# rareid2/Stanford_Raytracer

Hardware: AMD Instinct MI355X
Metric: ray-steps/sec (whole node) + achieved HBM GB/s vs roofline (higher is better)
Workload: dtype f64

## Files before the change

### stanford_raytracer_amd/csrc/srt_fastmath.hpp

```cpp
#pragma once
#include <hip/hip_runtime.h>

namespace srt {

constexpr double FM_PI = 3.14159265358979323846;

__device__ __forceinline__ double fdiv(double a, double b) {
  double r = __builtin_amdgcn_rcp(b);
  r = fma(fma(-b, r, 1.0), r, r);
  r = fma(fma(-b, r, 1.0), r, r);
  double q = a * r;
  return fma(fma(-b, q, a), r, q);
}

namespace fm {
__device__ __forceinline__ double sqrt_pos(double x) {
  const double y = __builtin_amdgcn_rsq(x);
  double g = x * y, h = 0.5 * y;
  const double r = fma(-h, g, 0.5);
  g = fma(g, r, g);
  h = fma(h, r, h);
  double d = fma(-g, g, x);
  g = fma(d, h, g);
  d = fma(-g, g, x);
  g = fma(d, h, g);
  return x == 0.0 ? 0.0 : g;
}
__device__ __forceinline__ void sqrt_and_inv_pos(double x, double &g_out, double &inv_out) {
  const double y = __builtin_amdgcn_rsq(x);
  double g = x * y, h = 0.5 * y;
  const double r = fma(-h, g, 0.5);
  g = fma(g, r, g);
  h = fma(h, r, h);
  double d = fma(-g, g, x);
  g = fma(d, h, g);
  d = fma(-g, g, x);
  g = fma(d, h, g);
  double inv = h + h;
  inv = fma(fma(-g, inv, 1.0), inv, inv);
  g_out = g;
  inv_out = inv;
}
__device__ __forceinline__ void sincos_0pi(double a, double &s, double &c) {
  const double PIO2_HI = 1.57079632673412561417e+00, PIO2_LO = 6.07710050650619224932e-11;
  const double kf = a > 0.75 * FM_PI ? 2.0 : (a > 0.25 * FM_PI ? 1.0 : 0.0);
  const double t = fma(-kf, PIO2_LO, fma(-kf, PIO2_HI, a));
  const double z = t * t;
  const double rs = 8.33333333332248946124e-03 + z * (-1.98412698298579493134e-04 + z * (2.75573137070700676789e-06 + z * (-2.50507602534068634195e-08 + z * 1.58969099521155010221e-10)));
  const double st = t + (z * t) * (-1.66666666666666324348e-01 + z * rs);
  const double rc = z * (4.16666666666666019037e-02 + z * (-1.38888888888741095749e-03 + z * (2.48015872894767294178e-05 + z * (-2.75573143513906633035e-07 + z * (2.08757232129817482790e-09 + z * -1.13596475577881948265e-11)))));
  const double hz = 0.5 * z, w = 1.0 - hz;
  const double ct = w + (((1.0 - w) - hz) + z * rc);
  s = kf == 1.0 ? ct : (kf == 2.0 ? -st : st);
  c = kf == 1.0 ? -st : (kf == 2.0 ? -ct : ct);
}
__device__ __forceinline__ double log_pos(double x) {
  double m = __builtin_amdgcn_frexp_mant(x);
  int e = __builtin_amdgcn_frexp_exp(x);
  const bool low = m < 0.70710678118654752440;
  m = low ? m + m : m;
  e = low ? e - 1 : e;
  const double f = m - 1.0, k = (double)e;
  const double sq = fdiv(f, 2.0 + f), z = sq * sq, w = z * z;
  const double t1 = w * (3.999999999940941908e-01 + w * (2.222219843214978396e-01 + w * 1.531383769920937332e-01));
  const double t2 = z * (6.666666666666735130e-01 + w * (2.857142874366239149e-01 + w * (1.818357216161805012e-01 + w * 1.479819860511658591e-01)));
  const double R = t2 + t1, hfsq = 0.5 * f * f;
  return k * 6.93147180369123816490e-01 - ((hfsq - (sq * (hfsq + R) + k * 1.90821492927058770002e-10)) - f);
}
__device__ __forceinline__ double exp_any(double y) {
  y = fmax(y, -800.0);
  const double k = rint(y * 1.44269504088896338700e+00);
  const double r = fma(-k, 1.90821492927058770002e-10, fma(-k, 6.93147180369123816490e-01, y));
  double p = 1.0 / 6227020800.0;
  p = fma(p, r, 1.0 / 479001600.0);
  p = fma(p, r, 1.0 / 39916800.0);
  p = fma(p, r, 1.0 / 3628800.0);
  p = fma(p, r, 1.0 / 362880.0);
  p = fma(p, r, 1.0 / 40320.0);
  p = fma(p, r, 1.0 / 5040.0);
  p = fma(p, r, 1.0 / 720.0);
  p = fma(p, r, 1.0 / 120.0);
  p = fma(p, r, 1.0 / 24.0);
  p = fma(p, r, 1.0 / 6.0);
  p = fma(p, r, 0.5);
  p = fma(p, r, 1.0);
  p = fma(p, r, 1.0);
  return ldexp(p, (int)k);
}
__device__ __forceinline__ void sincos_mod(double x, double &s, double &c) {
  const double k = rint(x * 0.63661977236758134308);
  double t = fma(-k, 1.57079632673412561417e+00, x);
  t = fma(-k, 6.07710050650619224932e-11, t);
  const double z = t * t;
  const double rs = 8.33333333332248946124e-03 + z * (-1.98412698298579493134e-04 + z * (2.75573137070700676789e-06 + z * (-2.50507602534068634195e-08 + z * 1.58969099521155010221e-10)));
  const double st = t + (z * t) * (-1.66666666666666324348e-01 + z * rs);
  const double rc = z * (4.16666666666666019037e-02 + z * (-1.38888888888741095749e-03 + z * (2.48015872894767294178e-05 + z * (-2.75573143513906633035e-07 + z * (2.08757232129817482790e-09 + z * -1.13596475577881948265e-11)))));
  const double hz = 0.5 * z, w = 1.0 - hz;
  const double ct = w + (((1.0 - w) - hz) + z * rc);
  const int q = (int)k;
  const double s1 = (q & 1) ? ct : st, c1 = (q & 1) ? -st : ct;
  s = (q & 2) ? -s1 : s1;
  c = (q & 2) ? -c1 : c1;
}
__device__ __forceinline__ double sin_mod(double x) {
  double s, c;
  sincos_mod(x, s, c);
  return s;
}
__device__ __forceinline__ double cos_mod(double x) {
  double s, c;
  sincos_mod(x, s, c);
  return c;
}
__device__ __forceinline__ double pow_pos(double x, double y) {
  if (!(x > 0.0) || !(x < 1.0e300)) return pow(x, y);
  return exp_any(y * log_pos(x));
}
}

}
```

### stanford_raytracer_amd/csrc/srt_models.hpp

```cpp
#pragma once
#include "srt_device.hpp"

namespace srt {

constexpr int WAVE = 64;
constexpr int UNIT_BYTES = WAVE * 128;
constexpr int RING = 4;
constexpr int TILE_PAD_BYTES = 2048;
constexpr int TILE_DOUBLES = (RING * UNIT_BYTES + TILE_PAD_BYTES) / 8;
constexpr int RES_CELL_BYTES = 0;
constexpr int RES_STATE_BYTES = WAVE * 4;
constexpr int RES_END_BYTES = RES_STATE_BYTES + WAVE * 4;
constexpr int MAX_UNIT_IMM = 384;
static_assert(RES_END_BYTES <= TILE_PAD_BYTES - MAX_UNIT_IMM, "the header must lie below every biased DMA base");
enum RingState : int { RING_INVALID = 0, RING_HOLDS_FIRST = 1, RING_HOLDS_LAST = 2 };

typedef double d2_t __attribute__((ext_vector_type(2)));
#ifdef SRT_TRIP_TIMING
constexpr int TT_SLOTS = 24;
__device__ unsigned long long srt_trip_cycles[TT_SLOTS];
__device__ __forceinline__ unsigned long long *srt_tt_lds() {
  __shared__ unsigned long long acc[TT_SLOTS];
  return acc;
}
#define SRT_LK_MARK(var_) __builtin_amdgcn_sched_barrier(0); const unsigned long long var_ = __builtin_readcyclecounter(); __builtin_amdgcn_sched_barrier(0)
#else
#define SRT_LK_MARK(var_) do {} while (0)
#endif

#ifdef SRT_PHASE_TIMING
__device__ unsigned long long srt_wave_stats[4] = {0ull, 0ull, ~0ull, 0ull};
#endif
template <class M>
__device__ __forceinline__ void bind_scratch(const M &, double *, double *, double * = nullptr) {}
template <class M>
__device__ __forceinline__ void new_ray_hook(const M &, double *, bool) {}
template <class M>
__device__ __forceinline__ void tile_reset(const M &, double *) {}
template <class M>
struct WaveBudget {
  static constexpr int LDS_DOUBLES = TILE_DOUBLES;
  static constexpr int WAVES_PER_EU = 1;
};
#define SRT_AS1 __attribute__((address_space(1)))
#define SRT_AS3 __attribute__((address_space(3)))

struct NgoModel {
  double r0, pi32;
  double therm, rbase, ane0, alpha0[5], rzero, scbot;
  double lk, expk, ddk, rconsn, scr;
  double l0[10], def[10], dd[10], rducln[10], rducun[10], rducls[10], rducus[10], sidedu[10];
  double hl2n[10], hl2s[10], hu2n[10], hu2s[10];
  int num, kducts, kinit;

  __device__ __noinline__ void dens_point(double x, double y, double z, double Ns[4]) const {
    double rho2 = x * x + y * y;
    double r2 = rho2 + z * z;
    double r = sqrt(r2);
    dens_core(r0 * r / R_E, rho2 / r2, z, Ns);
  }

  __device__ inline void dens_core(double z1, double sinz22, double latitu, double Ns[4]) const {
    double rb7370 = rbase / 7370.0;
    double sh2 = (double)1.150600f * therm * rb7370 * rb7370;
    double gph = rbase * (1.0 - rbase / z1);
    double e2 = exp(-gph / sh2);
    double e3 = e2 * e2 * e2 * e2;
    double e4 = e3 * e3 * e3 * e3;
    double q2 = alpha0[2] * e2, q3 = (num >= 3) ? alpha0[3] * e3 : 0.0, q4 = (num >= 4) ? alpha0[4] * e4 : 0.0;
    double q = q2 + q3 + q4;
    double anr = sqrt(q);
    double arg = (z1 - rzero) / scbot;
    if (!(arg < 13.0)) arg = 13.0;
    double anli = 1.0 - exp(-arg * arg);
    double l = z1 / (r0 * sinz22);
    double ani1 = ane0 * anr * anli;
    if (kducts != 0) {
      double deltal = l - lk;
      if (!(deltal < 0.0)) {
        double d2 = ddk * ddk;
        double argl = deltal * deltal / (d2 * 2.0);
        if (!(argl < 80.0)) argl = 80.0;
        double f = exp(-argl);
        double trm = pow(rconsn / z1, expk);
        double argr = (z1 - rconsn) / scr;
        if (!(argr < 12.5)) argr = 12.5;
        double fr = exp(-argr * argr);
        double trmodl = trm + (1.0 - trm) * fr;
        ani1 *= f + trmodl * (1.0 - f);
      }
      if (kducts != 1) ani1 *= ducts(l, z1, latitu);
    }
    double invq = 1.0 / q;
    Ns[0] = 1.0e6 * ani1;
    Ns[1] = 1.0e6 * (ani1 * (q2 * invq));
    Ns[2] = 1.0e6 * (ani1 * (q3 * invq));
    Ns[3] = 1.0e6 * (ani1 * (q4 * invq));
  }

  __device__ inline bool taper(int kd, double z1, double latitu, bool north_first, double &delnl) const {
    bool lower;
    if (north_first)
      lower = (latitu >= 0 && z1 <= rducun[kd]) || (latitu <= 0 && z1 <= rducus[kd]);
    else
      lower = (latitu <= 0 && z1 <= rducus[kd]) || (latitu >= 0 && z1 <= rducun[kd]);
    double delr = 0.0, arglr = 0.0;
    if (!lower) {
      if (north_first) {
        if (latitu >= 0) delr = z1 - rducun[kd];
        if (latitu <= 0) delr = z1 - rducus[kd];
        if (latitu >= 0) arglr = delr * delr / hu2n[kd];
        if (latitu <= 0) arglr = delr * delr / hu2s[kd];
      } else {
        if (latitu >= 0) delr = z1 - rducun[kd];
        if (latitu <= 0) delr = z1 - rducus[kd];
        if (latitu <= 0) arglr = delr * delr / hu2s[kd];
        if (latitu >= 0) arglr = delr * delr / hu2n[kd];
      }
      if (arglr >= 75.0) return false;
      delnl *= exp(-arglr);
      return true;
    }
    bool inside;
    if (north_first)
      inside = (latitu >= 0 && z1 >= rducln[kd]) || (latitu <= 0 && z1 >= rducls[kd]);
    else
      inside = (latitu <= 0 && z1 >= rducls[kd]) || (latitu >= 0 && z1 >= rducln[kd]);
    if (inside) return true;
    if (latitu >= 0) delr = z1 - rducln[kd];
    if (latitu <= 0) delr = z1 - rducls[kd];
    if (north_first) {
      if (latitu >= 0) arglr = delr * delr / hl2n[kd];
      if (latitu <= 0) arglr = delr * delr / hl2s[kd];
    } else {
      if (latitu <= 0) arglr = delr * delr / hl2s[kd];
      if (latitu >= 0) arglr = delr * delr / hl2n[kd];
    }
    if (arglr >= 75.0) return false;
    delnl *= exp(-arglr);
    return true;
  }

  __device__ __noinline__ double ducts(double l, double z1, double latitu) const {
    double fac = 1.0;
    int kstart = kinit;
    if (!(l0[2] > 0.0)) {
      kstart = 3;
      double dl = l + l0[2];
      if (!(dl * sidedu[2] >= 0.0)) dl = 0.0;
      double delk = -l0[2] - (lk + ddk) + dd[2] / 2;
      double critl = (lk + ddk) + fmod(delk, dd[2]);
      if (!(l <= critl)) {
        double argl = 2.0 * pi32 * dl / dd[2];
        double delnl = (def[2] / 2.0) * (1.0 + cos(argl));
        if (taper(2, z1, latitu, false, delnl)) fac *= 1.0 + delnl;
      }
      if (kducts == 2) return fac;
    }
    for (int kd = kstart; kd <= kducts; ++kd) {
      double dl = l - l0[kd];
      if (!(dl * sidedu[kd] >= 0.0)) dl = 0.0;
      double d2 = dd[kd] * dd[kd];
      double argl = dl * dl / (d2 * 2.0);
      if (argl > 80.0) continue;
      double delnl = def[kd] * exp(-argl);
      if (taper(kd, z1, latitu, true, delnl)) fac *= 1.0 + delnl;
    }
    return fac;
  }

  template <int NP>
  __device__ __forceinline__ void density(const double (&p)[NP][3], double (&Ns)[NP][4], double *) const {
#pragma unroll
    for (int i = 0; i < NP; ++i) dens_point(p[i][0], p[i][1], p[i][2], Ns[i]);
  }
  struct Dens2 {
    double a[4], b[4];
  };
  __device__ __noinline__ Dens2 dens_pair(double ax, double ay, double az, double bx, double by, double bz) const {
    Dens2 r;
    const double rhoa = ax * ax + ay * ay, ra2 = rhoa + az * az, ra = sqrt(ra2);
    const double rhob = bx * bx + by * by, rb2 = rhob + bz * bz, rb = sqrt(rb2);
    const double z1[2] = {r0 * ra / R_E, r0 * rb / R_E}, s2[2] = {rhoa / ra2, rhob / rb2}, lat[2] = {az, bz};
    double N[2][4];
    dens_core2(z1, s2, lat, N);
#pragma unroll
    for (int s = 0; s < 4; ++s) r.a[s] = N[0][s], r.b[s] = N[1][s];
    return r;
  }
  __device__ __forceinline__ void dens_core2(const double (&z1)[2], const double (&sinz22)[2], const double (&latitu)[2], double (&Ns)[2][4]) const {
    const double rb7370 = rbase / 7370.0;
    const double sh2 = (double)1.150600f * therm * rb7370 * rb7370;
    double q2[2], q3[2], q4[2], q[2], ani1[2], l[2];
#pragma unroll
    for (int p = 0; p < 2; ++p) {
      const double gph = rbase * (1.0 - rbase / z1[p]);
      const double e2 = exp(-gph / sh2);
      const double e3 = e2 * e2 * e2 * e2;
      const double e4 = e3 * e3 * e3 * e3;
      q2[p] = alpha0[2] * e2, q3[p] = (num >= 3) ? alpha0[3] * e3 : 0.0, q4[p] = (num >= 4) ? alpha0[4] * e4 : 0.0;
      q[p] = q2[p] + q3[p] + q4[p];
      const double anr = sqrt(q[p]);
      double arg = (z1[p] - rzero) / scbot;
      if (!(arg < 13.0)) arg = 13.0;
      const double anli = 1.0 - exp(-arg * arg);
      l[p] = z1[p] / (r0 * sinz22[p]);
      ani1[p] = ane0 * anr * anli;
    }
    if (kducts != 0) {
#pragma unroll
      for (int p = 0; p < 2; ++p) {
        const double deltal = l[p] - lk;
        const double d2 = ddk * ddk;
        double argl = deltal * deltal / (d2 * 2.0);
        if (!(argl < 80.0)) argl = 80.0;
        const double f = exp(-argl);
        const double trm = pow(rconsn / z1[p], expk);
        double argr = (z1[p] - rconsn) / scr;
        if (!(argr < 12.5)) argr = 12.5;
        const double fr = exp(-argr * argr);
        const double trmodl = trm + (1.0 - trm) * fr;
        const double with_pp = ani1[p] * (f + trmodl * (1.0 - f));
        ani1[p] = !(deltal < 0.0) ? with_pp : ani1[p];
      }
      if (kducts != 1) {
#pragma unroll
        for (int p = 0; p < 2; ++p) ani1[p] *= ducts(l[p], z1[p], latitu[p]);
      }
    }
#pragma unroll
    for (int p = 0; p < 2; ++p) {
      const double invq = 1.0 / q[p];
      Ns[p][0] = 1.0e6 * ani1[p];
      Ns[p][1] = 1.0e6 * (ani1[p] * (q2[p] * invq));
      Ns[p][2] = 1.0e6 * (ani1[p] * (q3[p] * invq));
      Ns[p][3] = 1.0e6 * (ani1[p] * (q4[p] * invq));
    }
  }
  template <int NE>
  __device__ __forceinline__ static void stencil_point(int i, const double oc[3], const double od[3], const double oe[3], double q[3]) {
#pragma unroll
    for (int a = 0; a < 3; ++a) {
      double v = oc[a];
      v = (i == 1 + 2 * a) ? oc[a] + od[a] : v;
      v = (i == 2 + 2 * a) ? oc[a] - od[a] : v;
      v = (NE && i == 7) ? oe[a] : v;
      q[a] = v;
    }
  }
  template <int NE>
  __device__ __forceinline__ void density_stencil(const double c[3], const double d[3], const double *extra,
                                                  double (&Ns)[7 + NE][4], double *, bool need = true) const {
    const unsigned long long needy = __ballot(need);
    const int nneedy = __popcll(needy);
    if (nneedy >= 1 && nneedy <= 16) {
#ifdef SRT_TRIP_TIMING
      __builtin_amdgcn_sched_barrier(0); unsigned long long tt0_ = __builtin_readcyclecounter(); __builtin_amdgcn_sched_barrier(0);
#define SRT_TTM(slot_) do { __builtin_amdgcn_sched_barrier(0); unsigned long long t1_ = __builtin_readcyclecounter(); __builtin_amdgcn_sched_barrier(0); if (threadIdx.x == 0) srt_tt_lds()[slot_] += t1_ - tt0_; tt0_ = t1_; } while (0)
#else
#define SRT_TTM(slot_) do {} while (0)
#endif
      const int lane = (int)__lane_id(), slot = lane >> 2, sub = lane & 3;
      unsigned long long mask = needy;
      for (int k = 0; k < slot && mask; ++k) mask &= mask - 1;
      const int owner = (slot < nneedy) ? __builtin_ctzll(mask) : lane;
      double oc[3], od[3], oe[3], qa[3], qb[3];
#pragma unroll
      for (int a = 0; a < 3; ++a) {
        oc[a] = __shfl(c[a], owner);
        od[a] = __shfl(d[a], owner);
        oe[a] = NE ? __shfl(extra[a], owner) : 0.0;
      }
      stencil_point<NE>(2 * sub, oc, od, oe, qa);
      stencil_point<NE>(2 * sub + 1, oc, od, oe, qb);
      SRT_TTM(11);
      const Dens2 mine = dens_pair(qa[0], qa[1], qa[2], qb[0], qb[1], qb[2]);
      SRT_TTM(12);
      const int rank = __popcll(needy & ((1ull << lane) - 1ull));
      __shared__ __attribute__((aligned(16))) double park[WAVE * 8];
      {
        d2_t *mp_ = (d2_t *)(park + 8 * lane);
        mp_[0] = d2_t{mine.a[0], mine.a[1]};
        mp_[1] = d2_t{mine.a[2], mine.a[3]};
        mp_[2] = d2_t{mine.b[0], mine.b[1]};
        mp_[3] = d2_t{mine.b[2], mine.b[3]};
      }
      __syncthreads();
#pragma unroll
      for (int i = 0; i < 7 + NE; ++i) {
        const d2_t *src = (const d2_t *)(park + 8 * ((4 * rank + (i >> 1)) & 63) + 4 * (i & 1));
        const d2_t u = src[0], v = src[1];
        Ns[i][0] = u.x, Ns[i][1] = u.y, Ns[i][2] = v.x, Ns[i][3] = v.y;
      }
      __syncthreads();
      SRT_TTM(13);
      return;
    }
    const double oe[3] = {NE ? extra[0] : 0.0, NE ? extra[1] : 0.0, NE ? extra[2] : 0.0};
#pragma unroll
    for (int h = 0; h < 4; ++h) {
      double qa[3], qb[3];
      stencil_point<NE>(2 * h, c, d, oe, qa);
      stencil_point<NE>(2 * h + 1, c, d, oe, qb);
      const Dens2 r = dens_pair(qa[0], qa[1], qa[2], qb[0], qb[1], qb[2]);
#pragma unroll
      for (int s = 0; s < 4; ++s) {
        Ns[2 * h][s] = r.a[s];
        if (2 * h + 1 < 7 + NE) Ns[2 * h + 1][s] = r.b[s];
      }
    }
  }
};

struct Axis {
  double min, del, rdel;
  int n;
  __device__ __forceinline__ double node(int i) const {
#pragma clang fp contract(off)
    double prod = (double)i * del;
    return prod + min;
  }
  __device__ __forceinline__ int locate(double xi, double &xl) const {
    double f = (xi - min) * rdel;
    int g;
    if (!(f >= 0.0)) g = 0;
    else if (f >= (double)n) g = n;
    else g = (int)f + 1;
    g += (g < n && node(g) <= xi) ? 1 : 0;
    g -= (g > 0 && node(g - 1) > xi) ? 1 : 0;
    xl = (g >= 1 && g < n) ? fdiv(xi - node(g - 1), del) : 0.0;
    return g;
  }
};

struct InterpModel {
  const double *coef;
  Axis ax, ay, az;
  int nspec;

  __device__ __forceinline__ int cell_id(int ci, int cj, int ck) const {
    return (ck * (ay.n + 1) + cj) * (ax.n + 1) + ci;
  }

  template <int NP, class Chunk>
  __device__ __forceinline__ static void eval(Chunk chunk, const double (&x)[NP], const double (&y)[NP],
                                              const double (&z)[NP], double (&out)[NP]) {
    double vz[NP];
#pragma unroll
    for (int i = 0; i < NP; ++i) vz[i] = 0.0;
#pragma unroll
    for (int k = 3; k >= 0; --k) {
      double vy[NP];
#pragma unroll
      for (int i = 0; i < NP; ++i) vy[i] = 0.0;
#pragma unroll
      for (int j = 3; j >= 0; --j) {
        const int q = 2 * j + 8 * k;
        double2 lo = chunk(q), hi = chunk(q + 1);
#pragma unroll
        for (int i = 0; i < NP; ++i) {
          double vx = fma(fma(fma(hi.y, x[i], hi.x), x[i], lo.y), x[i], lo.x);
          vy[i] = fma(vy[i], y[i], vx);
        }
      }
#pragma unroll
      for (int i = 0; i < NP; ++i) vz[i] = fma(vz[i], z[i], vy[i]);
    }
#pragma unroll
    for (int i = 0; i < NP; ++i) out[i] = vz[i];
  }

  template <bool EXP>
  __device__ __forceinline__ void point_direct_body(double x, double y, double z, double out[4]) const {
    double xl, yl, zl;
    int ci = ax.locate(x, xl), cj = ay.locate(y, yl), ck = az.locate(z, zl);
    const double *base = coef + (size_t)cell_id(ci, cj, ck) * (size_t)(nspec * 64);
#pragma unroll
    for (int s = 0; s < 4; ++s) {
      if (s < nspec) {
        const double2 *a = reinterpret_cast<const double2 *>(base + s * 64);
        double x1[1] = {xl}, y1[1] = {yl}, z1[1] = {zl}, o1[1];
        eval<1>([&](int q) { return a[q]; }, x1, y1, z1, o1);
        out[s] = EXP ? exp(o1[0]) : o1[0];
      } else if (EXP) out[s] = 0.0;
    }
  }
  __device__ __noinline__ void point_direct(double x, double y, double z, double lnN[4]) const { point_direct_body<false>(x, y, z, lnN); }
  __device__ __noinline__ void point_direct_exp(double x, double y, double z, double N[4]) const { point_direct_body<true>(x, y, z, N); }

  __device__ __forceinline__ void stage_prepare(int cell, unsigned long long (&a)[8], int species = 0) const {
    int lane = threadIdx.x;
    asm volatile("" : "+v"(lane));
    const unsigned long long base = reinterpret_cast<unsigned long long>(coef) +
                                    (unsigned long long)(unsigned)cell * (unsigned long long)(nspec * 512) + (unsigned)(species * 512);
    const int blo = (int)(unsigned)base, bhi = (int)(unsigned)(base >> 32);
    const int p = lane & 7, g = lane & 56;
#pragma unroll
    for (int t = 0; t < 8; ++t) {
      const int src = (g + t) << 2;
      const unsigned lo = (unsigned)__builtin_amdgcn_ds_bpermute(src, blo);
      const unsigned hi = (unsigned)__builtin_amdgcn_ds_bpermute(src, bhi);
      a[t] = (((unsigned long long)hi << 32) | (unsigned long long)lo) + (unsigned long long)(((p - t) & 7) << 4);
    }
  }
  __device__ __forceinline__ static void read_addrs(double *lds, unsigned (&ra)[8]) {
    int lane = threadIdx.x;
    asm volatile("" : "+v"(lane));
    const unsigned base = (unsigned)(unsigned long long)((SRT_AS3 char *)lds) + TILE_PAD_BYTES +
                          (unsigned)((8 * (lane & 7) + (lane >> 3)) * 128);
#pragma unroll
    for (int q = 0; q < 8; ++q) ra[q] = base + (unsigned)(((q + lane) & 7) << 4);
  }
  template <int IMM, int J, int AUX = 0>
  __device__ __forceinline__ static void issue_unit(const unsigned long long (&a)[8], double *lds) {
    static_assert(IMM <= MAX_UNIT_IMM, "the DMA base would reach into the residency header");
    SRT_AS3 char *ring = (SRT_AS3 char *)lds + TILE_PAD_BYTES;
#pragma unroll
    for (int t = 0; t < 8; ++t)
      __builtin_amdgcn_global_load_lds((const SRT_AS1 void *)a[t], (SRT_AS3 void *)(ring + (J * UNIT_BYTES + t * 1024 - IMM)),
                                       16, IMM, AUX);
  }
  __device__ __forceinline__ static void restage_issue(const unsigned long long (&a)[8], double *lds, unsigned long long miss) {
    SRT_AS3 char *ring = (SRT_AS3 char *)lds + TILE_PAD_BYTES;
    const unsigned owners = (unsigned)(miss >> (threadIdx.x & 56)) & 0xffu;
#pragma unroll
    for (int t = 0; t < 8; ++t) {
      if ((owners >> t) & 1u) {
        const SRT_AS1 void *src = (const SRT_AS1 void *)a[t];
        __builtin_amdgcn_global_load_lds(src, (SRT_AS3 void *)(ring + (0 * UNIT_BYTES + t * 1024 - 384)), 16, 384, 0);
        __builtin_amdgcn_global_load_lds(src, (SRT_AS3 void *)(ring + (1 * UNIT_BYTES + t * 1024 - 256)), 16, 256, 0);
        __builtin_amdgcn_global_load_lds(src, (SRT_AS3 void *)(ring + (2 * UNIT_BYTES + t * 1024 - 128)), 16, 128, 0);
        __builtin_amdgcn_global_load_lds(src, (SRT_AS3 void *)(ring + (3 * UNIT_BYTES + t * 1024)), 16, 0, 0);
      }
    }
  }
  __device__ __forceinline__ static unsigned res_addr(double *lds) {
    int lane = threadIdx.x;
    asm volatile("" : "+v"(lane));
    return (unsigned)(unsigned long long)((SRT_AS3 char *)lds) + (unsigned)(RES_CELL_BYTES + 4 * lane);
  }
  __device__ __forceinline__ static void ring_read(double *lds, int &state, int &held) {
    asm volatile("ds_read_b32 %0, %2 offset:%3\n\t"
                 "ds_read_b32 %1, %2\n\t"
                 "s_waitcnt lgkmcnt(0)"
                 : "=&v"(state), "=&v"(held)
                 : "v"(res_addr(lds)), "n"(RES_STATE_BYTES - RES_CELL_BYTES)
                 : "memory");
    state = __builtin_amdgcn_readfirstlane(state);
  }
  __device__ __forceinline__ static void ring_write_state(double *lds, int state) {
    asm volatile("ds_write_b32 %0, %1 offset:%2" ::"v"(res_addr(lds)), "v"(state), "n"(RES_STATE_BYTES - RES_CELL_BYTES) : "memory");
  }
  __device__ __forceinline__ static void ring_write_cell(double *lds, int cell) {
    asm volatile("ds_write_b32 %0, %1" ::"v"(res_addr(lds)), "v"(cell) : "memory");
  }
  template <int N>
  __device__ __forceinline__ static void wait_vm() {
    asm volatile("s_waitcnt vmcnt(%0)" ::"n"(N) : "memory");
  }
  template <int J>
  __device__ __forceinline__ static void read_unit(const unsigned (&ra)[8], d2_t (&c)[8]) {
    asm volatile("ds_read_b128 %0, %8 offset:%16\n\t"
                 "ds_read_b128 %1, %9 offset:%16\n\t"
                 "ds_read_b128 %2, %10 offset:%16\n\t"
                 "ds_read_b128 %3, %11 offset:%16\n\t"
                 "ds_read_b128 %4, %12 offset:%16\n\t"
                 "ds_read_b128 %5, %13 offset:%16\n\t"
                 "ds_read_b128 %6, %14 offset:%16\n\t"
                 "ds_read_b128 %7, %15 offset:%16\n\t"
                 "s_waitcnt lgkmcnt(0)"
                 : "=&v"(c[0]), "=&v"(c[1]), "=&v"(c[2]), "=&v"(c[3]), "=&v"(c[4]), "=&v"(c[5]), "=&v"(c[6]), "=&v"(c[7])
                 : "v"(ra[0]), "v"(ra[1]), "v"(ra[2]), "v"(ra[3]), "v"(ra[4]), "v"(ra[5]), "v"(ra[6]), "v"(ra[7]),
                   "n"(J * UNIT_BYTES)
                 : "memory");
  }

  template <int NE>
  __device__ __forceinline__ static void plane_stencil(const d2_t (&c)[8], const double (&X)[3], const double (&Y)[3],
                                                       const double (&Z)[3], const double (&E)[3],
                                                       double (&vz)[7 + NE]) {
    double vc = 0.0, vxp = 0.0, vxm = 0.0, vyp = 0.0, vym = 0.0, ve = 0.0;
#pragma unroll
    for (int j = 3; j >= 0; --j) {
      const d2_t lo = c[2 * j], hi = c[2 * j + 1];
      double h0 = fma(fma(fma(hi.y, X[0], hi.x), X[0], lo.y), X[0], lo.x);
      double hp = fma(fma(fma(hi.y, X[1], hi.x), X[1], lo.y), X[1], lo.x);
      double hm = fma(fma(fma(hi.y, X[2], hi.x), X[2], lo.y), X[2], lo.x);
      vc = fma(vc, Y[0], h0);
      vxp = fma(vxp, Y[0], hp);
      vxm = fma(vxm, Y[0], hm);
      vyp = fma(vyp, Y[1], h0);
      vym = fma(vym, Y[2], h0);
      if (NE) {
        double he = fma(fma(fma(hi.y, E[0], hi.x), E[0], lo.y), E[0], lo.x);
        ve = fma(ve, E[1], he);
      }
    }
    vz[0] = fma(vz[0], Z[0], vc);
    vz[1] = fma(vz[1], Z[0], vxp);
    vz[2] = fma(vz[2], Z[0], vxm);
    vz[3] = fma(vz[3], Z[0], vyp);
    vz[4] = fma(vz[4], Z[0], vym);
    vz[5] = fma(vz[5], Z[1], vc);
    vz[6] = fma(vz[6], Z[2], vc);
    if (NE) vz[7 + NE - 1] = fma(vz[7 + NE - 1], E[2], ve);
  }
  template <int NP>
  __device__ __forceinline__ static void plane_points(const d2_t (&c)[8], const double (&x)[NP], const double (&y)[NP],
                                                      const double (&z)[NP], double (&vz)[NP]) {
    double vy[NP];
#pragma unroll
    for (int i = 0; i < NP; ++i) vy[i] = 0.0;
#pragma unroll
    for (int j = 3; j >= 0; --j) {
      const d2_t lo = c[2 * j], hi = c[2 * j + 1];
#pragma unroll
      for (int i = 0; i < NP; ++i) {
        double vx = fma(fma(fma(hi.y, x[i], hi.x), x[i], lo.y), x[i], lo.x);
        vy[i] = fma(vy[i], y[i], vx);
      }
    }
#pragma unroll
    for (int i = 0; i < NP; ++i) vz[i] = fma(vz[i], z[i], vy[i]);
  }

  template <int NE>
  __device__ __forceinline__ void density_stencil(const double c[3], const double d[3], const double *extra,
                                                  double (&Ns)[7 + NE][4], double *lds, bool = true) const {
    SRT_LK_MARK(lk0_);
    double X[3], Y[3], Z[3], E[3] = {0.0, 0.0, 0.0};
    const int ci = ax.locate(c[0], X[0]), cj = ay.locate(c[1], Y[0]), ck = az.locate(c[2], Z[0]);
    const int cell = cell_id(ci, cj, ck);
    int state, held;
    ring_read(lds, state, held);
    const bool desc = state == RING_HOLDS_LAST;
    const unsigned long long miss = __ballot(state == RING_INVALID || held != cell);
#ifdef SRT_TRIP_TIMING
    if (threadIdx.x == 0) srt_tt_lds()[14] += (unsigned long long)__popcll(miss), srt_tt_lds()[15] += miss ? 1ull : 0ull;
#endif
    ring_write_cell(lds, cell);
    ring_write_state(lds, desc ? RING_HOLDS_FIRST : RING_HOLDS_LAST);
    unsigned long long a[8];
    unsigned ra[8];
    stage_prepare(cell, a, desc ? nspec - 1 : 0);
    read_addrs(lds, ra);
    const unsigned long long step = desc ? (unsigned long long)-512ll : 512ull;
    SRT_LK_MARK(lk1_);
    if (miss) restage_issue(a, lds, miss);
    SRT_LK_MARK(lk2_);
    double dd[3] = {d[0], d[1], d[2]}, ee[3] = {NE ? extra[0] : 0.0, NE ? extra[1] : 0.0, NE ? extra[2] : 0.0};
#pragma unroll
    for (int a_ = 0; a_ < 3; ++a_) {
      asm volatile("" : "+v"(dd[a_]));
      if (NE) asm volatile("" : "+v"(ee[a_]));
    }
    bool same = true;
    same = same && (ax.locate(c[0] + dd[0], X[1]) == ci) && (ax.locate(c[0] - dd[0], X[2]) == ci);
    same = same && (ay.locate(c[1] + dd[1], Y[1]) == cj) && (ay.locate(c[1] - dd[1], Y[2]) == cj);
    same = same && (az.locate(c[2] + dd[2], Z[1]) == ck) && (az.locate(c[2] - dd[2], Z[2]) == ck);
    bool extra_same = true;
    if (NE) {
      extra_same = (ax.locate(ee[0], E[0]) == ci) && (ay.locate(ee[1], E[1]) == cj) && (az.locate(ee[2], E[2]) == ck);
    }
    SRT_LK_MARK(lk3_);
    wait_vm<0>();
    SRT_LK_MARK(lk4_);
#pragma unroll
    for (int t = 0; t < 8; ++t) a[t] += step;
    double acc[7 + NE][4];
#pragma unroll
    for (int i = 0; i < 7 + NE; ++i)
#pragma unroll
      for (int k = 0; k < 4; ++k) acc[i][k] = 0.0;
#pragma unroll 1
    for (int s = 0; s < nspec; ++s) {
      const bool more = s + 1 < nspec;
      const int sp = desc ? nspec - 1 - s : s;
      double vz[7 + NE];
#pragma unroll
      for (int i = 0; i < 7 + NE; ++i) vz[i] = 0.0;
      d2_t cf[8];
      wait_vm<24>();
      read_unit<0>(ra, cf);
      plane_stencil<NE>(cf, X, Y, Z, E, vz);
      if (more) {
        issue_unit<384, 0>(a, lds);
        wait_vm<24>();
      } else wait_vm<16>();
      read_unit<1>(ra, cf);
      plane_stencil<NE>(cf, X, Y, Z, E, vz);
      if (more) {
        issue_unit<256, 1>(a, lds);
        wait_vm<24>();
      } else wait_vm<8>();
      read_unit<2>(ra, cf);
      plane_stencil<NE>(cf, X, Y, Z, E, vz);
      if (more) {
        issue_unit<128, 2>(a, lds);
        wait_vm<24>();
      } else wait_vm<0>();
      read_unit<3>(ra, cf);
      plane_stencil<NE>(cf, X, Y, Z, E, vz);
      if (more) issue_unit<0, 3>(a, lds);
#pragma unroll
      for (int t = 0; t < 8; ++t) a[t] += step;
#pragma unroll
      for (int i = 0; i < 7 + NE; ++i) {
        const double e = exp(vz[i]);
#pragma unroll
        for (int k = 0; k < 4; ++k) acc[i][k] = (k == sp) ? e : acc[i][k];
      }
    }
    SRT_LK_MARK(lk5_);
    wait_vm<0>();
    if (__any(!same || !extra_same)) {
      if (!same) {
#pragma unroll
        for (int ax_ = 0; ax_ < 3; ++ax_)
#pragma unroll
          for (int sg = 0; sg < 2; ++sg) {
            double pt[3] = {c[0], c[1], c[2]}, t[4];
            pt[ax_] = sg ? c[ax_] - d[ax_] : c[ax_] + d[ax_];
            point_direct_exp(pt[0], pt[1], pt[2], t);
#pragma unroll
            for (int k = 0; k < 4; ++k) acc[1 + 2 * ax_ + sg][k] = t[k];
          }
      }
      if (NE && !extra_same) {
        double t[4];
        point_direct_exp(extra[0], extra[1], extra[2], t);
#pragma unroll
        for (int k = 0; k < 4; ++k) acc[7 + NE - 1][k] = t[k];
      }
    }
#pragma unroll
    for (int i = 0; i < 7 + NE; ++i)
#pragma unroll
      for (int k = 0; k < 4; ++k) Ns[i][k] = acc[i][k];
#ifdef SRT_TRIP_TIMING
    SRT_LK_MARK(lk6_);
    if (threadIdx.x == 0) {
      unsigned long long *tt_ = srt_tt_lds();
      tt_[16] += lk1_ - lk0_, tt_[17] += lk2_ - lk1_, tt_[18] += lk3_ - lk2_, tt_[19] += lk4_ - lk3_, tt_[20] += lk5_ - lk4_;
      tt_[21] += lk6_ - lk5_, tt_[22] += 1ull;
    }
#endif
  }

  template <int NP>
  __device__ __forceinline__ void density(const double (&p)[NP][3], double (&Ns)[NP][4], double *lds) const {
    double xl[NP], yl[NP], zl[NP];
    int ci = ax.locate(p[0][0], xl[0]);
    int cj = ay.locate(p[0][1], yl[0]);
    int ck = az.locate(p[0][2], zl[0]);
    unsigned strag = 0;
#pragma unroll
    for (int i = 1; i < NP; ++i) {
      int c1 = ax.locate(p[i][0], xl[i]);
      int c2 = ay.locate(p[i][1], yl[i]);
      int c3 = az.locate(p[i][2], zl[i]);
      if (c1 != ci || c2 != cj || c3 != ck) strag |= 1u << i;
    }
    unsigned long long a[8];
    unsigned ra[8];
    ring_write_state(lds, RING_INVALID);
    stage_prepare(cell_id(ci, cj, ck), a);
    read_addrs(lds, ra);
    double acc[NP][4];
#pragma unroll
    for (int i = 0; i < NP; ++i)
#pragma unroll
      for (int k = 0; k < 4; ++k) acc[i][k] = 0.0;
#pragma unroll 1
    for (int s = 0; s < nspec; ++s) {
      double vz[NP];
#pragma unroll
      for (int i = 0; i < NP; ++i) vz[i] = 0.0;
      d2_t cf[8];
      issue_unit<384, 0>(a, lds);
      issue_unit<256, 1>(a, lds);
      issue_unit<128, 2>(a, lds);
      issue_unit<0, 3>(a, lds);
      wait_vm<0>();
      read_unit<0>(ra, cf);
      plane_points<NP>(cf, xl, yl, zl, vz);
      read_unit<1>(ra, cf);
      plane_points<NP>(cf, xl, yl, zl, vz);
      read_unit<2>(ra, cf);
      plane_points<NP>(cf, xl, yl, zl, vz);
      read_unit<3>(ra, cf);
      plane_points<NP>(cf, xl, yl, zl, vz);
#pragma unroll
      for (int i = 0; i < NP; ++i)
#pragma unroll
        for (int k = 0; k < 4; ++k) acc[i][k] = (k == s) ? vz[i] : acc[i][k];
#pragma unroll
      for (int t = 0; t < 8; ++t) a[t] += 512;
    }
    if (__any(strag != 0)) {
#pragma unroll
      for (int i = 1; i < NP; ++i)
        if (strag & (1u << i)) {
          double t[4] = {0.0, 0.0, 0.0, 0.0};
          point_direct(p[i][0], p[i][1], p[i][2], t);
#pragma unroll
          for (int k = 0; k < 4; ++k) acc[i][k] = t[k];
        }
    }
#pragma unroll
    for (int i = 0; i < NP; ++i)
#pragma unroll
      for (int s = 0; s < 4; ++s) Ns[i][s] = (s < nspec) ? exp(acc[i][s]) : 0.0;
  }
};
__device__ __forceinline__ void tile_reset(const InterpModel &, double *lds) { InterpModel::ring_write_state(lds, RING_INVALID); }
__device__ __forceinline__ void new_ray_hook(const InterpModel &, double *lds, bool) { InterpModel::ring_write_cell(lds, -1); }

}
```

Baseline: 640.5 million.

## Double-buffer LDS unit reads and replace neighbor locate calls with in-cell checks

The per-species stencil loop now issues the LDS reads for the next unit into a second register buffer before running the current plane stencil, and waits on lgkmcnt instead of blocking each read. This is meant to hide LDS latency and to reissue global DMA earlier. The neighbor points are now tested against the centre cell's bounds with branchless in_cell checks, and each axis uses a hoisted wave-uniform reciprocal of del, in place of six or more full locate calls with divisions. Trip-timing counters are added for the new wait spans. The cost is higher register pressure from the extra d2_t buffer, and the inline-asm pins may constrain scheduling.

After: 707.3 million (median of 6 runs). 1.1x the previous value.

```diff
diff --git a/stanford_raytracer_amd/csrc/srt_fastmath.hpp b/stanford_raytracer_amd/csrc/srt_fastmath.hpp
--- a/stanford_raytracer_amd/csrc/srt_fastmath.hpp
+++ b/stanford_raytracer_amd/csrc/srt_fastmath.hpp
@@ -5,13 +5,17 @@
 
 constexpr double FM_PI = 3.14159265358979323846;
 
-__device__ __forceinline__ double fdiv(double a, double b) {
+__device__ __forceinline__ double fdiv_recip(double b) {
   double r = __builtin_amdgcn_rcp(b);
   r = fma(fma(-b, r, 1.0), r, r);
   r = fma(fma(-b, r, 1.0), r, r);
+  return r;
+}
+__device__ __forceinline__ double fdiv_r(double a, double b, double r) {
   double q = a * r;
   return fma(fma(-b, q, a), r, q);
 }
+__device__ __forceinline__ double fdiv(double a, double b) { return fdiv_r(a, b, fdiv_recip(b)); }
 
 namespace fm {
 __device__ __forceinline__ double sqrt_pos(double x) {
diff --git a/stanford_raytracer_amd/csrc/srt_models.hpp b/stanford_raytracer_amd/csrc/srt_models.hpp
--- a/stanford_raytracer_amd/csrc/srt_models.hpp
+++ b/stanford_raytracer_amd/csrc/srt_models.hpp
@@ -17,15 +17,21 @@
 
 typedef double d2_t __attribute__((ext_vector_type(2)));
 #ifdef SRT_TRIP_TIMING
-constexpr int TT_SLOTS = 24;
+constexpr int TT_SLOTS = 26;
 __device__ unsigned long long srt_trip_cycles[TT_SLOTS];
 __device__ __forceinline__ unsigned long long *srt_tt_lds() {
   __shared__ unsigned long long acc[TT_SLOTS];
   return acc;
 }
 #define SRT_LK_MARK(var_) __builtin_amdgcn_sched_barrier(0); const unsigned long long var_ = __builtin_readcyclecounter(); __builtin_amdgcn_sched_barrier(0)
+#define SRT_LK_SUMS() unsigned long long lkrd_ = 0ull, lkvm_ = 0ull, lks0_ = 0ull
+#define SRT_LK_SPAN_BEGIN() do { __builtin_amdgcn_sched_barrier(0); lks0_ = __builtin_readcyclecounter(); __builtin_amdgcn_sched_barrier(0); } while (0)
+#define SRT_LK_SPAN_END(sum_) do { __builtin_amdgcn_sched_barrier(0); sum_ += __builtin_readcyclecounter() - lks0_; __builtin_amdgcn_sched_barrier(0); } while (0)
 #else
 #define SRT_LK_MARK(var_) do {} while (0)
+#define SRT_LK_SUMS() do {} while (0)
+#define SRT_LK_SPAN_BEGIN() do {} while (0)
+#define SRT_LK_SPAN_END(sum_) do {} while (0)
 #endif
 
 #ifdef SRT_PHASE_TIMING
@@ -321,15 +327,26 @@
     return prod + min;
   }
   __device__ __forceinline__ int locate(double xi, double &xl) const {
-    double f = (xi - min) * rdel;
-    int g;
-    if (!(f >= 0.0)) g = 0;
-    else if (f >= (double)n) g = n;
-    else g = (int)f + 1;
-    g += (g < n && node(g) <= xi) ? 1 : 0;
-    g -= (g > 0 && node(g - 1) > xi) ? 1 : 0;
-    xl = (g >= 1 && g < n) ? fdiv(xi - node(g - 1), del) : 0.0;
+    double lo;
+    return locate(xi, xl, fdiv_recip(del), lo);
+  }
+  __device__ __forceinline__ int locate(double xi, double &xl, double r, double &lo) const {
+    const double f = (xi - min) * rdel;
+    const double fc = fmin(fmax(f, 0.0), (double)n);
+    int g = (int)fc + 1;
+    g = (f >= (double)n) ? n : g;
+    g = !(f >= 0.0) ? 0 : g;
+    g += (int)((g < n) & (node(g) <= xi));
+    g -= (int)((g > 0) & (node(g - 1) > xi));
+    lo = node(g - 1);
+    xl = ((g >= 1) & (g < n)) ? fdiv_r(xi - lo, del, r) : 0.0;
     return g;
+  }
+  __device__ __forceinline__ bool in_cell(double xi, int g, double lo, double hi, double r, double &xl) const {
+    const bool below_hi = (g < n) ? !(hi <= xi) : true;
+    const bool above_lo = (g > 0) ? (xi >= lo) : true;
+    xl = ((g >= 1) & (g < n)) ? fdiv_r(xi - lo, del, r) : 0.0;
+    return below_hi & above_lo;
   }
 };
 
@@ -338,9 +355,8 @@
   Axis ax, ay, az;
   int nspec;
 
-  __device__ __forceinline__ int cell_id(int ci, int cj, int ck) const {
-    return (ck * (ay.n + 1) + cj) * (ax.n + 1) + ci;
-  }
+  __device__ __forceinline__ static int cell_id(int nx, int ny, int ci, int cj, int ck) { return (ck * (ny + 1) + cj) * (nx + 1) + ci; }
+  __device__ __forceinline__ int cell_id(int ci, int cj, int ck) const { return cell_id(ax.n, ay.n, ci, cj, ck); }
 
   template <int NP, class Chunk>
   __device__ __forceinline__ static void eval(Chunk chunk, const double (&x)[NP], const double (&y)[NP],
@@ -453,6 +469,12 @@
   }
   __device__ __forceinline__ static void ring_write_cell(double *lds, int cell) {
     asm volatile("ds_write_b32 %0, %1" ::"v"(res_addr(lds)), "v"(cell) : "memory");
+  }
+  __device__ __forceinline__ static double uniform(double v) {
+    const unsigned long long u = (unsigned long long)__double_as_longlong(v);
+    const unsigned lo = (unsigned)__builtin_amdgcn_readfirstlane((int)(unsigned)u);
+    const unsigned hi = (unsigned)__builtin_amdgcn_readfirstlane((int)(unsigned)(u >> 32));
+    return __longlong_as_double((long long)(((unsigned long long)hi << 32) | lo));
   }
   template <int N>
   __device__ __forceinline__ static void wait_vm() {
@@ -475,6 +497,29 @@
                  : "memory");
   }
 
+  template <int J>
+  __device__ __forceinline__ static void read_unit_issue(const unsigned (&ra)[8], d2_t (&c)[8]) {
+    asm volatile("ds_read_b128 %6, %14 offset:%16\n\t"
+                 "ds_read_b128 %7, %15 offset:%16\n\t"
+                 "ds_read_b128 %4, %12 offset:%16\n\t"
+                 "ds_read_b128 %5, %13 offset:%16\n\t"
+                 "ds_read_b128 %2, %10 offset:%16\n\t"
+                 "ds_read_b128 %3, %11 offset:%16\n\t"
+                 "ds_read_b128 %0, %8 offset:%16\n\t"
+                 "ds_read_b128 %1, %9 offset:%16"
+                 : "=&v"(c[0]), "=&v"(c[1]), "=&v"(c[2]), "=&v"(c[3]), "=&v"(c[4]), "=&v"(c[5]), "=&v"(c[6]), "=&v"(c[7])
+                 : "v"(ra[0]), "v"(ra[1]), "v"(ra[2]), "v"(ra[3]), "v"(ra[4]), "v"(ra[5]), "v"(ra[6]), "v"(ra[7]),
+                   "n"(J * UNIT_BYTES)
+                 : "memory");
+  }
+  template <int N>
+  __device__ __forceinline__ static void wait_lgkm(d2_t (&c)[8]) {
+    asm volatile("s_waitcnt lgkmcnt(%8)"
+                 : "+v"(c[0]), "+v"(c[1]), "+v"(c[2]), "+v"(c[3]), "+v"(c[4]), "+v"(c[5]), "+v"(c[6]), "+v"(c[7])
+                 : "n"(N)
+                 : "memory");
+  }
+
   template <int NE>
   __device__ __forceinline__ static void plane_stencil(const d2_t (&c)[8], const double (&X)[3], const double (&Y)[3],
                                                        const double (&Z)[3], const double (&E)[3],
@@ -529,8 +574,11 @@
                                                   double (&Ns)[7 + NE][4], double *lds, bool = true) const {
     SRT_LK_MARK(lk0_);
     double X[3], Y[3], Z[3], E[3] = {0.0, 0.0, 0.0};
-    const int ci = ax.locate(c[0], X[0]), cj = ay.locate(c[1], Y[0]), ck = az.locate(c[2], Z[0]);
-    const int cell = cell_id(ci, cj, ck);
+    const Axis lx = ax, ly = ay, lz = az;
+    const double rx = uniform(fdiv_recip(lx.del)), ry = uniform(fdiv_recip(ly.del)), rz = uniform(fdiv_recip(lz.del));
+    double xlo, ylo, zlo;
+    const int ci = lx.locate(c[0], X[0], rx, xlo), cj = ly.locate(c[1], Y[0], ry, ylo), ck = lz.locate(c[2], Z[0], rz, zlo);
+    const int cell = cell_id(lx.n, ly.n, ci, cj, ck);
     int state, held;
     ring_read(lds, state, held);
     const bool desc = state == RING_HOLDS_LAST;
@@ -554,14 +602,18 @@
       asm volatile("" : "+v"(dd[a_]));
       if (NE) asm volatile("" : "+v"(ee[a_]));
     }
-    bool same = true;
-    same = same && (ax.locate(c[0] + dd[0], X[1]) == ci) && (ax.locate(c[0] - dd[0], X[2]) == ci);
-    same = same && (ay.locate(c[1] + dd[1], Y[1]) == cj) && (ay.locate(c[1] - dd[1], Y[2]) == cj);
-    same = same && (az.locate(c[2] + dd[2], Z[1]) == ck) && (az.locate(c[2] - dd[2], Z[2]) == ck);
+    const double xhi = lx.node(ci), yhi = ly.node(cj), zhi = lz.node(ck);
+    const bool same = lx.in_cell(c[0] + dd[0], ci, xlo, xhi, rx, X[1]) & lx.in_cell(c[0] - dd[0], ci, xlo, xhi, rx, X[2]) &
+                      ly.in_cell(c[1] + dd[1], cj, ylo, yhi, ry, Y[1]) & ly.in_cell(c[1] - dd[1], cj, ylo, yhi, ry, Y[2]) &
+                      lz.in_cell(c[2] + dd[2], ck, zlo, zhi, rz, Z[1]) & lz.in_cell(c[2] - dd[2], ck, zlo, zhi, rz, Z[2]);
     bool extra_same = true;
     if (NE) {
-      extra_same = (ax.locate(ee[0], E[0]) == ci) && (ay.locate(ee[1], E[1]) == cj) && (az.locate(ee[2], E[2]) == ck);
-    }
+      extra_same = lx.in_cell(ee[0], ci, xlo, xhi, rx, E[0]) & ly.in_cell(ee[1], cj, ylo, yhi, ry, E[1]) &
+                   lz.in_cell(ee[2], ck, zlo, zhi, rz, E[2]);
+    }
+    unsigned away = (same ? 0u : 1u) | (extra_same ? 0u : 2u);
+    asm volatile("" : "+v"(away), "+v"(X[1]), "+v"(X[2]), "+v"(Y[1]), "+v"(Y[2]), "+v"(Z[1]), "+v"(Z[2]));
+    if (NE) asm volatile("" : "+v"(E[0]), "+v"(E[1]), "+v"(E[2]));
     SRT_LK_MARK(lk3_);
     wait_vm<0>();
     SRT_LK_MARK(lk4_);
@@ -572,6 +624,7 @@
     for (int i = 0; i < 7 + NE; ++i)
 #pragma unroll
       for (int k = 0; k < 4; ++k) acc[i][k] = 0.0;
+    SRT_LK_SUMS();
 #pragma unroll 1
     for (int s = 0; s < nspec; ++s) {
       const bool more = s + 1 < nspec;
@@ -580,28 +633,36 @@
 #pragma unroll
       for (int i = 0; i < 7 + NE; ++i) vz[i] = 0.0;
       d2_t cf[8];
-      wait_vm<24>();
-      read_unit<0>(ra, cf);
+#define SRT_LOOP_WAIT_VM(n_) do { SRT_LK_SPAN_BEGIN(); wait_vm<n_>(); SRT_LK_SPAN_END(lkvm_); } while (0)
+#define SRT_LOOP_PIN_VZ() do { asm volatile("" : "+v"(vz[0]), "+v"(vz[1]), "+v"(vz[2]), "+v"(vz[3]), "+v"(vz[4]), "+v"(vz[5]), "+v"(vz[6])); if (NE) asm volatile("" : "+v"(vz[7 + NE - 1])); } while (0)
+      d2_t cg[8];
+      SRT_LOOP_WAIT_VM(24);
+      read_unit_issue<0>(ra, cf);
+      SRT_LOOP_WAIT_VM(16);
+      read_unit_issue<1>(ra, cg);
+      SRT_LK_SPAN_BEGIN(); wait_lgkm<8>(cf); SRT_LK_SPAN_END(lkrd_);
+      if (more) issue_unit<384, 0>(a, lds);
       plane_stencil<NE>(cf, X, Y, Z, E, vz);
-      if (more) {
-        issue_unit<384, 0>(a, lds);
-        wait_vm<24>();
-      } else wait_vm<16>();
-      read_unit<1>(ra, cf);
+      SRT_LOOP_PIN_VZ();
+      if (more) SRT_LOOP_WAIT_VM(16);
+      else SRT_LOOP_WAIT_VM(8);
+      read_unit_issue<2>(ra, cf);
+      SRT_LK_SPAN_BEGIN(); wait_lgkm<8>(cg); SRT_LK_SPAN_END(lkrd_);
+      if (more) issue_unit<256, 1>(a, lds);
+      plane_stencil<NE>(cg, X, Y, Z, E, vz);
+      SRT_LOOP_PIN_VZ();
+      if (more) SRT_LOOP_WAIT_VM(16);
+      else SRT_LOOP_WAIT_VM(0);
+      read_unit_issue<3>(ra, cg);
+      SRT_LK_SPAN_BEGIN(); wait_lgkm<8>(cf); SRT_LK_SPAN_END(lkrd_);
+      if (more) issue_unit<128, 2>(a, lds);
       plane_stencil<NE>(cf, X, Y, Z, E, vz);
-      if (more) {
-        issue_unit<256, 1>(a, lds);
-        wait_vm<24>();
-      } else wait_vm<8>();
-      read_unit<2>(ra, cf);
-      plane_stencil<NE>(cf, X, Y, Z, E, vz);
-      if (more) {
-        issue_unit<128, 2>(a, lds);
-        wait_vm<24>();
-      } else wait_vm<0>();
-      read_unit<3>(ra, cf);
-      plane_stencil<NE>(cf, X, Y, Z, E, vz);
+      SRT_LOOP_PIN_VZ();
+      SRT_LK_SPAN_BEGIN(); wait_lgkm<0>(cg); SRT_LK_SPAN_END(lkrd_);
       if (more) issue_unit<0, 3>(a, lds);
+      plane_stencil<NE>(cg, X, Y, Z, E, vz);
+#undef SRT_LOOP_WAIT_VM
+#undef SRT_LOOP_PIN_VZ
 #pragma unroll
       for (int t = 0; t < 8; ++t) a[t] += step;
 #pragma unroll
@@ -613,8 +674,8 @@
     }
     SRT_LK_MARK(lk5_);
     wait_vm<0>();
-    if (__any(!same || !extra_same)) {
-      if (!same) {
+    if (__any(away != 0u)) {
+      if (away & 1u) {
 #pragma unroll
         for (int ax_ = 0; ax_ < 3; ++ax_)
 #pragma unroll
@@ -626,7 +687,7 @@
             for (int k = 0; k < 4; ++k) acc[1 + 2 * ax_ + sg][k] = t[k];
           }
       }
-      if (NE && !extra_same) {
+      if (NE && (away & 2u)) {
         double t[4];
         point_direct_exp(extra[0], extra[1], extra[2], t);
 #pragma unroll
@@ -643,6 +704,7 @@
       unsigned long long *tt_ = srt_tt_lds();
       tt_[16] += lk1_ - lk0_, tt_[17] += lk2_ - lk1_, tt_[18] += lk3_ - lk2_, tt_[19] += lk4_ - lk3_, tt_[20] += lk5_ - lk4_;
       tt_[21] += lk6_ - lk5_, tt_[22] += 1ull;
+      tt_[24] += lkrd_, tt_[25] += lkvm_;
     }
 #endif
   }
```
